# tum-vision/mem

Hardware: AMD Instinct MI355X
Metric: pretrain samples/sec (ViT-B, 224^2 event voxels) (higher is better)
Workload: dtype bf16

## Files before the change

include/memhip.h:

```cpp
#ifndef MEMHIP_H
#define MEMHIP_H

#include <stddef.h>
#include <stdint.h>

#ifdef __cplusplus
extern "C" {
#endif

#define MEMHIP_ABI_VERSION 7

#define MEMHIP_OK 0
#define MEMHIP_EINVAL (-1)
#define MEMHIP_EWORKSPACE (-2)
#define MEMHIP_ELAUNCH (-3)
#define MEMHIP_EUNSUPPORTED (-4)

typedef void* memhip_stream_t;

int memhip_abi_version(void);
const char* memhip_last_error(void);
const char* memhip_arch(void);
const char* memhip_build_flags(void);
int memhip_set_option(const char* name, int value);
// ... 126 lines not shown

#define MEMHIP_NT_128 0
#define MEMHIP_NT_G256 1
#define MEMHIP_NT_P8_256 2
#define MEMHIP_NT_P8_128 3
#define MEMHIP_NT_P8_PAIR 4
typedef struct memhip_nt_launch {
  int32_t kind;
  int32_t row0, rows;
  int32_t tail_rows;
  int32_t guard;
  int32_t copy;
  int32_t grid, tail_grid;
} memhip_nt_launch_t;
typedef struct memhip_nt_plan { int32_t count; memhip_nt_launch_t l[2]; } memhip_nt_plan_t;
int memhip_gemm_bf16_nt_plan(const memhip_gemm_args_t* args, int stream_cus, int device_cus, memhip_nt_plan_t* out);

int memhip_gemm_bf16_tn(const void* A, int64_t lda, const void* B, int64_t ldb, int R, int N, int K,
                        float* out, int64_t ldo, int accumulate, memhip_stream_t stream);
size_t memhip_gemm_bf16_tn_workspace(int R, int N, int K);
int memhip_gemm_bf16_tn_ws(const void* A, int64_t lda, const void* B, int64_t ldb, int R, int N, int K,
                           float* out, int64_t ldo, int accumulate, void* workspace, size_t workspace_bytes,
                           memhip_stream_t stream);
typedef struct memhip_tn_problem {
  const void* A; int64_t lda;
  const void* B; int64_t ldb;
  float* out; int64_t ldo;
  int32_t R, N, K;
  int32_t reserved0;
} memhip_tn_problem_t;
size_t memhip_gemm_bf16_tn_group_workspace(const memhip_tn_problem_t* problems, int count);
int memhip_gemm_bf16_tn_group(const memhip_tn_problem_t* problems, int count, int accumulate, void* workspace,
                              size_t workspace_bytes, memhip_stream_t stream);
int memhip_colsum_bf16(const void* in, int64_t ld, int R, int C, float* out, memhip_stream_t stream);
int memhip_colsum_fold(float* ws, int copies, int N, float* out, memhip_stream_t stream);

int memhip_residual_rows(const float* x, int64_t ldx, const int32_t* rows, const void* y, int64_t ldy, const float* gamma,
                         const float* rowkeep, float keep_prob, int R, int D, float* out, int64_t ldo,
                         memhip_stream_t stream);
int memhip_scatter_rows_f32(const float* src, int64_t lds, const int32_t* rows, int R, int D, float* dst, int64_t ldd,
                            memhip_stream_t stream);

int memhip_layernorm_fwd(const float* x, int64_t ldx, const int32_t* row_idx, int R, int D,
                         const float* gamma, const float* beta, float eps, void* y_bf16, int64_t ldy,
                         float* mean, float* rstd, memhip_stream_t stream);
int memhip_layernorm_bwd(const void* dy_bf16, int64_t lddy, const float* x, int64_t ldx,
                         const int32_t* row_idx, int R, int D, const float* gamma, const float* mean,
                         const float* rstd, float* dres, int64_t lddres, int accumulate, float* dgamma,
                         float* dbeta, memhip_stream_t stream);

int memhip_layerscale_grad(const void* W_bf16, int64_t ldw, const float* dW, int64_t lddw, const float* bias,
                           const float* dbias, const float* gamma, int N, int K, float* dgamma,
                           memhip_stream_t stream);

int memhip_layernorm_bwd_branch(const void* dy_bf16, int64_t lddy, const float* x, int64_t ldx, int R, int D,
                                const float* gamma, const float* mean, const float* rstd, float* dres,
                                int64_t lddres, float* dgamma, float* dbeta, const void* y_branch_bf16, int64_t ldyb,
                                const float* gamma_branch, const float* rowmask, float keep_prob,
                                int rows_per_sample, void* dy_branch_bf16, int64_t lddyb, float* dgamma_branch,
                                float* dbias_branch, memhip_stream_t stream);

int memhip_branch_bwd(const float* dx, int64_t lddx, const void* y_bf16, int64_t ldy, const float* gamma,
                      const float* rowmask, float keep_prob, int rows_per_sample, int M, int D,
                      void* dy_bf16, int64_t lddy, float* dgamma, float* dbias, memhip_stream_t stream);
int memhip_branch_bwd_map(const float* dx, int64_t lddx, const void* y_bf16, int64_t ldy, const float* gamma,
                          const float* rowmask, float keep_prob, int rows_per_sample, int M, int D,
// ... 170 lines not shown
```

mem_amd/csrc/common.h:

```cpp
#pragma once
#include <hip/hip_runtime.h>
#include <cstdarg>
#include <cstdio>
#include <cstdint>
#include "../../include/memhip.h"

namespace memhip {

extern thread_local char g_err[512];

inline int fail(int code, const char* fmt, ...) {
  va_list ap;
  va_start(ap, fmt);
  vsnprintf(g_err, sizeof(g_err), fmt, ap);
  va_end(ap);
  return code;
}

inline int check_launch(const char* what) {
  hipError_t e = hipGetLastError();
  if (e != hipSuccess) return fail(MEMHIP_ELAUNCH, "%s: %s", what, hipGetErrorString(e));
  return MEMHIP_OK;
}

enum { OPT_GEMM_P8, OPT_GEMM256, OPT_GEMM_SPLIT, OPT_GEMM_P8_HALF, OPT_GEMM_P8_MIN_N, OPT_GEMM256_MIN_N, OPT_TN_P8,
       OPT_RASTER_LDS, OPT_ATTN16, OPT_ATTN16_STAGGER, OPT_ATTN16_STAGGER_FWD, OPT_GEMM_STAGGER, OPT_GEMM_PREFETCH, OPT_RESERVE_CUS, OPT_LN_BWD_GRID, OPT_ATTN_WIN, OPT_GEMM_P8_PAIR, OPT_TN_GROUP, OPT_CONV_WAVES, OPT_RASTER_BANDS, OPT_COUNT_ };
int opt(int id);
int usable_cus(hipStream_t s = nullptr);
int max_cus();

inline hipStream_t as_stream(memhip_stream_t s) { return reinterpret_cast<hipStream_t>(s); }

inline int cdiv(long long a, long long b) { return (int)((a + b - 1) / b); }

}

#define MEMHIP_REQUIRE(cond, ...) \
  do { if (!(cond)) return memhip::fail(MEMHIP_EINVAL, __VA_ARGS__); } while (0)
#define MEMHIP_HIP(call) \
  do { hipError_t e_ = (call); if (e_ != hipSuccess) \
    return memhip::fail(MEMHIP_ELAUNCH, "%s: %s", #call, hipGetErrorString(e_)); } while (0)
```

mem_amd/csrc/core.cpp:

```cpp
#include "common.h"
#include <atomic>
#include <mutex>
#include <cstring>

namespace memhip {
thread_local char g_err[512] = "";

static std::atomic<int> g_opt[OPT_COUNT_] = {
     {1},  {1},  {1},  {1},  {512},
     {1024},  {1},  {1},  {1},  {40000},  {0},  {0},  {0},
     {0},  {2048},
     {1},
     {1},
     {1},
     {16},
     {0}};
static const char* const g_opt_name[OPT_COUNT_] = {"gemm_p8", "gemm256", "gemm_split", "gemm_p8_half", "gemm_p8_min_n",
                                                   "gemm256_min_n", "tn_p8", "raster_lds", "attn16", "attn16_stagger", "attn16_stagger_fwd", "gemm_stagger", "gemm_prefetch", "reserve_cus", "ln_bwd_grid", "attn_win", "gemm_p8_pair", "tn_group", "conv_waves", "raster_bands"};
int opt(int id) { return g_opt[id].load(std::memory_order_relaxed); }

struct StreamReserve { std::atomic<bool> used{false}; std::atomic<void*> stream{nullptr}; std::atomic<int> cus{0}; };
static StreamReserve g_reserve[32];
static int stream_reserved(hipStream_t s) {
  for (auto& r : g_reserve)
    if (r.used.load(std::memory_order_acquire) && r.stream.load(std::memory_order_relaxed) == (void*)s)
      return r.cus.load(std::memory_order_relaxed);
  return 0;
}

static int device_cu_count() {
  static std::atomic<int> device_cus{0};
  int n = device_cus.load(std::memory_order_relaxed);
  if (!n) {
    int dev = 0;
    hipDeviceProp_t prop;
    if (hipGetDevice(&dev) != hipSuccess || hipGetDeviceProperties(&prop, dev) != hipSuccess) return 0;
    n = prop.multiProcessorCount > 0 ? prop.multiProcessorCount : 256;
    device_cus.store(n, std::memory_order_relaxed);
  }
  return n;
}

int max_cus() { return device_cu_count(); }

int usable_cus(hipStream_t s) {
  const int n = device_cu_count();
  if (!n) return 0;
  int r = opt(OPT_RESERVE_CUS);
  const int rs = stream_reserved(s);
  r = r > rs ? r : rs;
  r = r < 0 ? 0 : (r + 7) / 8 * 8;
// ... 58 lines not shown
```

mem_amd/csrc/gemm_tn_p8.hip:

```cpp
#include <atomic>
#include "common.h"

#define P8_PRIO_MODE 0
#define P8_PRIO(x) __builtin_amdgcn_s_setprio(x)

namespace {

using namespace memhip;

constexpr int BM = 256, BN = 256, BR = 64;
constexpr int kThreads = 512;
constexpr int kHalf = BR * 128 * 2;
constexpr int kBuf = 4 * kHalf;
constexpr int kRing = 2 * kBuf;
enum { HA0 = 0, HA1 = 1, HB0 = 2, HB1 = 3 };

typedef __attribute__((ext_vector_type(8))) __bf16 bf16x8;
typedef __attribute__((ext_vector_type(4))) short s16x4;
typedef __attribute__((ext_vector_type(4))) float f32x4;
typedef __attribute__((ext_vector_type(16))) float f32x16;

__device__ __attribute__((aligned(256))) unsigned char g_tnp8_zero[256];
#ifdef P8_STAMP
__device__ unsigned long long g_tnp8_stamps[256 * 4];
#endif

__device__ __forceinline__ void glds16(const void* gsrc, void* lds_dst) {
  __builtin_amdgcn_global_load_lds((const __attribute__((address_space(1))) void*)gsrc,
                                   (__attribute__((address_space(3))) void*)lds_dst, 16, 0, 0);
}
#define P8_SADDR 1
__device__ __forceinline__ void glds16s(const void* sbase, unsigned voff, const void* lds_dst) {
  const unsigned lds = (unsigned)(unsigned long long)((const __attribute__((address_space(3))) char*)lds_dst);
  asm volatile("s_mov_b32 m0, %2\n\ts_nop 0\n\tglobal_load_lds_dwordx4 %0, %1" ::"v"(voff), "s"(sbase), "s"(lds) : "memory", "m0");
}
template <int OFF>
__device__ __forceinline__ s16x4 lds_tr16_b64(unsigned lds_addr) {
  s16x4 r;
  asm volatile("ds_read_b64_tr_b16 %0, %1 offset:%2" : "=v"(r) : "v"(lds_addr), "n"(OFF) : "memory");
  return r;
}
template <int OFF>
__device__ __forceinline__ bf16x8 tr_pair(unsigned lds_addr) {
  union { struct { s16x4 l, h; } s; bf16x8 v; } u;
  u.s.l = lds_tr16_b64<OFF>(lds_addr);
  u.s.h = lds_tr16_b64<OFF + 16 * 256>(lds_addr);
  return u.v;
}

#define TP_WAIT_VM() asm volatile("s_waitcnt vmcnt(10)" ::: "memory")
#define TP_BARRIER()                      \
  do {                                    \
    __builtin_amdgcn_sched_barrier(0);    \
    __builtin_amdgcn_s_barrier();         \
    __builtin_amdgcn_sched_barrier(0);    \
  } while (0)

__device__ __forceinline__ int tn_xcd_wid() {
  const int gq = (int)gridDim.x / 8, gr = (int)gridDim.x % 8, xcd = (int)blockIdx.x % 8;
  return (xcd < gr ? xcd * (gq + 1) : gr * (gq + 1) + (xcd - gr) * gq) + (int)blockIdx.x / 8;
}

template <bool WS>
__device__ __forceinline__ void tn_p8_body(const __bf16* __restrict__ A, long long lda, const __bf16* __restrict__ B,
                                           long long ldb, int R, int N, int K, float* __restrict__ out, long long ldo,
                                           int rows_per_split, int wid) {
  extern __shared__ __attribute__((aligned(16))) char smem[];
  const int lane = threadIdx.x & 63;
  const int wave = __builtin_amdgcn_readfirstlane(threadIdx.x >> 6);
  const int wr = wave >> 2, wc = wave & 3;
  const int ntk = K / BN;
  const int tiles = (N / BM) * ntk;
  const int tile = wid % tiles, sp = wid / tiles;
  const int n0 = (tile / ntk) * BM, k0 = (tile % ntk) * BN;
  const int rbeg = sp * rows_per_split;
  int rend = rbeg + rows_per_split;
  rend = rend < R ? rend : R;
  if (rbeg >= rend) return;
  const int total = ((rend - rbeg + 2 * BR - 1) / (2 * BR)) * 2;

  int prow[2];
  unsigned offA[2], offB[2];
  const int cpos = lane & 15;
#pragma unroll
  for (int j = 0; j < 2; ++j) {
    prow[j] = (wave * 2 + j) * 4 + (lane >> 4);
    const unsigned chunk = (unsigned)((((cpos >> 1) ^ (prow[j] & 7)) << 1) | (cpos & 1));
    offA[j] = (unsigned)((long long)prow[j] * lda * 2) + chunk * 16;
    offB[j] = (unsigned)((long long)prow[j] * ldb * 2) + chunk * 16;
  }
  const char* zsrc = reinterpret_cast<const char*>(g_tnp8_zero) + cpos * 16;
  auto stage = [&](int H, int buf, int g) {
    char* slot = smem + buf * kBuf + H * kHalf + wave * 2048;
    const int r0 = rbeg + g * BR;
    const bool isA = H == HA0 || H == HA1;
    const int c0 = (isA ? n0 : k0) + ((H == HA1 || H == HB1) ? 128 : 0);
    const char* base = reinterpret_cast<const char*>(isA ? A : B) + ((long long)r0 * (isA ? lda : ldb) + c0) * 2;
    if (r0 + BR <= rend) {
#pragma unroll
      for (int j = 0; j < 2; ++j) {
        if (P8_SADDR) glds16s(base, isA ? offA[j] : offB[j], slot + j * 1024);
        else glds16(base + (isA ? offA[j] : offB[j]), slot + j * 1024);
      }
    } else {
#pragma unroll
      for (int j = 0; j < 2; ++j) {
        const char* src = (r0 + prow[j] < rend) ? base + (isA ? offA[j] : offB[j]) : zsrc;
        glds16(src, slot + j * 1024);
      }
    }
  };
// ... 80 lines not shown
    TP_MFMA(2, bq0);                                                                                      \
    TP_BARRIER();                                                                                         \
  } while (0)

  TP_READ_B(bx, 0, 0);
#ifdef P8_STAMP
  if (wave == 0) {
    unsigned long long t_, r_;
    asm volatile("s_memtime %0\n\ts_memrealtime %1\n\ts_waitcnt lgkmcnt(0)" : "=s"(t_), "=s"(r_)::"memory");
    if (lane == 0) { g_tnp8_stamps[(blockIdx.x & 255) * 4 + 0] = t_; g_tnp8_stamps[(blockIdx.x & 255) * 4 + 1] = r_; }
  }
#endif
  for (int c = 0; c < total; c += 2) {
    {
      constexpr int bc = 0;
      TP_KTILE(bx, by);
    }
    {
      constexpr int bc = 1;
      TP_KTILE(by, bx);
    }
  }
#ifdef P8_STAMP
  if (wave == 0) {
    unsigned long long t_, r_;
    asm volatile("s_memtime %0\n\ts_memrealtime %1\n\ts_waitcnt lgkmcnt(0)" : "=s"(t_), "=s"(r_)::"memory");
    if (lane == 0) { g_tnp8_stamps[(blockIdx.x & 255) * 4 + 2] = t_; g_tnp8_stamps[(blockIdx.x & 255) * 4 + 3] = r_; }
  }
#endif
  if (wr == 0) TP_BARRIER();
  asm volatile("s_waitcnt vmcnt(0)" ::: "memory");
  TP_BARRIER();

  float* wreg = reinterpret_cast<float*>(smem + wave * 4096);
  const int kcol = k0 + (lane >> 5) * 128 + wc * 32 + (lane & 31);
  float* dst = WS ? out + (long long)sp * N * ldo : out;
#pragma unroll
  for (int i = 0; i < 2; ++i)
#pragma unroll
    for (int nf = 0; nf < 4; ++nf) {
#pragma unroll
      for (int j = 0; j < 2; ++j)
#pragma unroll
        for (int kf = 0; kf < 2; ++kf)
#pragma unroll
          for (int r = 0; r < 4; ++r) {
            const int row = (lane >> 4) * 4 + r;
            wreg[row * 64 + ((j * 32 + kf * 16 + (lane & 15)) ^ (((row >> 2) & 1) << 4))] = TP_ACC_EL(i * 2 + j, nf, kf, r);
          }
      const int nrow = n0 + i * 128 + wr * 64 + nf * 16;
      if constexpr (WS) {
#pragma unroll
        for (int it = 0; it < 4; ++it) {
          const int row = it * 4 + (lane >> 4), c4 = (lane & 15) * 4;
          *reinterpret_cast<float4*>(dst + (long long)(nrow + row) * ldo + k0 + (c4 >> 5) * 128 + wc * 32 + (c4 & 31)) =
              *reinterpret_cast<const float4*>(wreg + row * 64 + (c4 ^ (((row >> 2) & 1) << 4)));
        }
      } else {
#pragma unroll
        for (int row = 0; row < 16; ++row) {
          const float v = wreg[row * 64 + (lane ^ (((row >> 2) & 1) << 4))];
          atomicAdd(dst + (long long)(nrow + row) * ldo + kcol, v);
        }
      }
    }
}

template <bool WS>
__global__ __launch_bounds__(kThreads) void gemm_tn_p8_kernel(const __bf16* __restrict__ A, long long lda,
                                                              const __bf16* __restrict__ B, long long ldb,
                                                              int R, int N, int K, float* __restrict__ out,
                                                              long long ldo, int rows_per_split) {
  tn_p8_body<WS>(A, lda, B, ldb, R, N, K, out, ldo, rows_per_split, tn_xcd_wid());
}

constexpr int kTnGroupMax = 4;
struct TnGroupProblem {
  const __bf16* A;
  const __bf16* B;
  float* ws;
  float* out;
  long long lda, ldb, ldo;
  int R, N, K;
  int rows_per_split, splits;
  int wg_begin;
  int quad_begin;
};
struct TnGroup {
  TnGroupProblem p[kTnGroupMax];
  int count;
};
__global__ __launch_bounds__(kThreads) void gemm_tn_p8_group_kernel(const TnGroup g) {
  const int wid = tn_xcd_wid();
  int i = 0;
#pragma unroll
  for (int j = 1; j < kTnGroupMax; ++j)
    if (j < g.count && wid >= g.p[j].wg_begin) i = j;
  const TnGroupProblem& q = g.p[i];
  tn_p8_body<true>(q.A, q.lda, q.B, q.ldb, q.R, q.N, q.K, q.ws, (long long)q.K, q.rows_per_split, wid - q.wg_begin);
}
__global__ __launch_bounds__(256) void tn_reduce_group_kernel(const TnGroup g, int accumulate) {
  const int quad = blockIdx.x * 256 + threadIdx.x;
  int i = 0;
#pragma unroll
  for (int j = 1; j < kTnGroupMax; ++j)
    if (j < g.count && quad >= g.p[j].quad_begin) i = j;
  const TnGroupProblem& q = g.p[i];
  const long long i4 = (long long)(quad - q.quad_begin) * 4;
  const long long slab = (long long)q.N * q.K;
  if (i4 >= slab) return;
  float4 a = *reinterpret_cast<const float4*>(q.ws + i4);
  for (int s = 1; s < q.splits; ++s) {
    const float4 b = *reinterpret_cast<const float4*>(q.ws + s * slab + i4);
    a.x += b.x; a.y += b.y; a.z += b.z; a.w += b.w;
  }
  const long long n = i4 / q.K, k = i4 - n * q.K;
  float4* o = reinterpret_cast<float4*>(q.out + n * q.ldo + k);
  if (accumulate) {
    const float4 c = *o;
    a.x += c.x; a.y += c.y; a.z += c.z; a.w += c.w;
  }
  *o = a;
}

__global__ __launch_bounds__(256) void tn_reduce_kernel(const float* __restrict__ ws, int S, long long slab, int N, int K,
                                                        float* __restrict__ out, long long ldo, int accumulate) {
  const long long i4 = ((long long)blockIdx.x * 256 + threadIdx.x) * 4;
  if (i4 >= (long long)N * K) return;
  float4 a = *reinterpret_cast<const float4*>(ws + i4);
  for (int s = 1; s < S; ++s) {
    const float4 b = *reinterpret_cast<const float4*>(ws + s * slab + i4);
    a.x += b.x; a.y += b.y; a.z += b.z; a.w += b.w;
  }
  const long long n = i4 / K, k = i4 - n * K;
  float4* o = reinterpret_cast<float4*>(out + n * ldo + k);
  if (accumulate) {
    const float4 c = *o;
    a.x += c.x; a.y += c.y; a.z += c.z; a.w += c.w;
  }
  *o = a;
}

}

#ifdef P8_STAMP
extern "C" int memhip_debug_tnp8_stamps(unsigned long long* host_out) {
  return hipMemcpyFromSymbol(host_out, HIP_SYMBOL(g_tnp8_stamps), sizeof(unsigned long long) * 256 * 4) == hipSuccess ? 0 : -1;
}
#endif

namespace memhip {

static void tn_p8_plan(int R, int N, int K, int num_cu, int& tiles, int& splits, int& rows_per_split) {
  tiles = (N / BM) * (K / BN);
  const int pairs = cdiv(R, 2 * BR);
  splits = num_cu / tiles;
  if (splits < 1) splits = 1;
  if (splits > pairs / 2) splits = pairs / 2 > 0 ? pairs / 2 : 1;
  rows_per_split = cdiv(pairs, splits) * 2 * BR;
  splits = cdiv(R, rows_per_split);
}
static int tn_p8_num_cu(hipStream_t s = nullptr) { return usable_cus(s); }

size_t gemm_tn_p8_workspace(int R, int N, int K) {
  if (N % BM != 0 || K % BN != 0 || R < 2048) return 0;
  const int num_cu = max_cus();
  if (!num_cu) return 0;
  size_t need = 0;
  for (int cu = num_cu; cu >= 8; cu -= 8) {
    int tiles, splits, rps;
    tn_p8_plan(R, N, K, cu, tiles, splits, rps);
    const size_t b = splits > 1 ? (size_t)splits * N * K * sizeof(float) : 0;
    need = b > need ? b : need;
  }
  return need;
}

int gemm_tn_p8_dispatch(const void* A, long long lda, const void* B, long long ldb, int R, int N, int K, float* out,
                        long long ldo, int accumulate, float* ws, size_t ws_bytes, hipStream_t s) {
  if (N % BM != 0 || K % BN != 0 || R < 2048) return MEMHIP_EUNSUPPORTED;
  const int num_cu = tn_p8_num_cu(s);
  if (!num_cu) return MEMHIP_EUNSUPPORTED;
  int tiles, splits, rows_per_split;
  tn_p8_plan(R, N, K, num_cu, tiles, splits, rows_per_split);
  static std::atomic<bool> attr_done{false};
  if (!attr_done) {
    hipError_t e = hipFuncSetAttribute(reinterpret_cast<const void*>(gemm_tn_p8_kernel<false>),
                                       hipFuncAttributeMaxDynamicSharedMemorySize, kRing);
    if (e == hipSuccess)
      e = hipFuncSetAttribute(reinterpret_cast<const void*>(gemm_tn_p8_kernel<true>),
                              hipFuncAttributeMaxDynamicSharedMemorySize, kRing);
    if (e != hipSuccess) return fail(MEMHIP_ELAUNCH, "gemm_tn_p8: set smem attr: %s", hipGetErrorString(e));
    attr_done = true;
  }
  const size_t need = (size_t)splits * N * K * sizeof(float);
  if (ws && splits > 1 && ws_bytes >= need && ((uintptr_t)ws & 15) == 0 && ldo % 4 == 0 && ((uintptr_t)out & 15) == 0) {
    hipLaunchKernelGGL(gemm_tn_p8_kernel<true>, dim3(tiles * splits), dim3(kThreads), kRing, s, (const __bf16*)A, lda,
                       (const __bf16*)B, ldb, R, N, K, ws, (long long)K, rows_per_split);
    const long long quads = (long long)N * K / 4;
    hipLaunchKernelGGL(tn_reduce_kernel, dim3((unsigned)((quads + 255) / 256)), dim3(256), 0, s, ws, splits,
                       (long long)N * K, N, K, out, ldo, accumulate);
    return check_launch("gemm_bf16_tn(p8, workspace)");
  }
  if (!accumulate) {
    hipError_t e = hipMemset2DAsync(out, (size_t)ldo * sizeof(float), 0, (size_t)K * sizeof(float), (size_t)N, s);
    if (e != hipSuccess) return fail(MEMHIP_ELAUNCH, "gemm_tn_p8: memset: %s", hipGetErrorString(e));
  }
  hipLaunchKernelGGL(gemm_tn_p8_kernel<false>, dim3(tiles * splits), dim3(kThreads), kRing, s, (const __bf16*)A, lda,
                     (const __bf16*)B, ldb, R, N, K, out, ldo, rows_per_split);
  return check_launch("gemm_bf16_tn(p8)");
}

static bool tn_group_plan(const memhip_tn_problem_t* pr, int count, int num_cu, TnGroup& g, int& total_wgs, int& total_quads,
                          size_t& ws_floats) {
  if (count < 2 || count > kTnGroupMax || !num_cu) return false;
  int tiles_total = 0;
  for (int i = 0; i < count; ++i) {
    if (pr[i].N % BM != 0 || pr[i].K % BN != 0 || pr[i].R < 2048 || pr[i].ldo % 4 != 0 || ((uintptr_t)pr[i].out & 15) != 0) return false;
    tiles_total += (pr[i].N / BM) * (pr[i].K / BN);
  }
  int best_s = 0;
  double best_eff = 0.0;
  for (int r = 1; r <= 4; ++r) {
    const int sp = (r * num_cu) / tiles_total;
    if (sp < 2) continue;
    const double eff = (double)tiles_total * sp / ((double)r * num_cu);
    if (eff > best_eff + 1e-9) { best_eff = eff; best_s = sp; }
    if (eff >= 0.80) break;
  }
  if (best_s < 2) return false;
  total_wgs = 0; total_quads = 0; ws_floats = 0;
  g.count = count;
  for (int i = 0; i < count; ++i) {
    TnGroupProblem& q = g.p[i];
    const int tiles = (pr[i].N / BM) * (pr[i].K / BN);
    const int pairs = cdiv(pr[i].R, 2 * BR);
    int sp = best_s;
    if (sp > pairs / 2) sp = pairs / 2 > 0 ? pairs / 2 : 1;
    q.rows_per_split = cdiv(pairs, sp) * 2 * BR;
    q.splits = cdiv(pr[i].R, q.rows_per_split);
    q.A = (const __bf16*)pr[i].A; q.B = (const __bf16*)pr[i].B;
    q.lda = pr[i].lda; q.ldb = pr[i].ldb; q.ldo = pr[i].ldo;
    q.R = pr[i].R; q.N = pr[i].N; q.K = pr[i].K;
    q.out = pr[i].out;
    q.ws = nullptr;
    q.wg_begin = total_wgs;
    q.quad_begin = total_quads;
    total_wgs += tiles * q.splits;
    total_quads += (int)(((long long)pr[i].N * pr[i].K / 4 + 255) / 256 * 256);
    ws_floats += (size_t)q.splits * pr[i].N * pr[i].K;
  }
  return true;
}

size_t gemm_tn_p8_group_workspace(const memhip_tn_problem_t* pr, int count) {
  const int num_cu = max_cus();
  size_t need = 0;
  for (int cu = num_cu; cu >= 8; cu -= 8) {
    TnGroup g;
    int wgs, quads;
    size_t fl;
    if (tn_group_plan(pr, count, cu, g, wgs, quads, fl) && fl * sizeof(float) > need) need = fl * sizeof(float);
  }
  return need;
}

int gemm_tn_p8_group_dispatch(const memhip_tn_problem_t* pr, int count, int accumulate, float* ws, size_t ws_bytes, hipStream_t s) {
  TnGroup g;
  int wgs, quads;
  size_t fl;
  if (!ws || ((uintptr_t)ws & 15) != 0 || !tn_group_plan(pr, count, tn_p8_num_cu(s), g, wgs, quads, fl) ||
      fl * sizeof(float) > ws_bytes)
    return MEMHIP_EUNSUPPORTED;
  static std::atomic<bool> attr_done{false};
  if (!attr_done) {
    const hipError_t e = hipFuncSetAttribute(reinterpret_cast<const void*>(gemm_tn_p8_group_kernel),
                                             hipFuncAttributeMaxDynamicSharedMemorySize, kRing);
    if (e != hipSuccess) return fail(MEMHIP_ELAUNCH, "gemm_tn_p8(group): set smem attr: %s", hipGetErrorString(e));
    attr_done = true;
  }
  float* w = ws;
  for (int i = 0; i < count; ++i) {
    g.p[i].ws = w;
    w += (size_t)g.p[i].splits * g.p[i].N * g.p[i].K;
  }
  hipLaunchKernelGGL(gemm_tn_p8_group_kernel, dim3(wgs), dim3(kThreads), kRing, s, g);
  hipLaunchKernelGGL(tn_reduce_group_kernel, dim3((unsigned)(quads / 256)), dim3(256), 0, s, g, accumulate);
  return check_launch("gemm_bf16_tn_group(p8)");
}

}
```

Measured before the change: 7484.

## Schedule TN weight-gradient GEMM work from a host-built segment table

Replaces the fixed split-K grouping of TN (weight-gradient) GEMMs with a host-side planner. The planner emits a per-workgroup table of (product, tile, row range, slot) segments, which is cached per shape set and uploaded to the device once. Each workgroup can now process several segments and writes partial results into per-slot tile buffers. A table-driven reduction then sums each tile's slots. An optional 'even' mode (off by default) balances row-pair work across CUs exactly, while the default slice mode reproduces the old split scheme through the table. The cost is an extra table lookup and an indirection in the reduce.

```diff
diff --git a/include/memhip.h b/include/memhip.h
--- a/include/memhip.h
+++ b/include/memhip.h
@@ -182,6 +182,10 @@
 size_t memhip_gemm_bf16_tn_group_workspace(const memhip_tn_problem_t* problems, int count);
 int memhip_gemm_bf16_tn_group(const memhip_tn_problem_t* problems, int count, int accumulate, void* workspace,
                               size_t workspace_bytes, memhip_stream_t stream);
+typedef struct memhip_tn_segment { int32_t wg, product, tile, pair_begin, pair_end, slot; } memhip_tn_segment_t;
+typedef struct memhip_tn_tile_slots { int32_t product, tile, first_slot, count; } memhip_tn_tile_slots_t;
+int memhip_gemm_bf16_tn_plan(const int32_t* shapes, int count, int cus, int even, memhip_tn_segment_t* segments, int segment_cap,
+                             memhip_tn_tile_slots_t* tiles, int tile_cap, int32_t* info);
 int memhip_colsum_bf16(const void* in, int64_t ld, int R, int C, float* out, memhip_stream_t stream);
 int memhip_colsum_fold(float* ws, int copies, int N, float* out, memhip_stream_t stream);
 
diff --git a/mem_amd/csrc/common.h b/mem_amd/csrc/common.h
--- a/mem_amd/csrc/common.h
+++ b/mem_amd/csrc/common.h
@@ -24,7 +24,7 @@
 }
 
 enum { OPT_GEMM_P8, OPT_GEMM256, OPT_GEMM_SPLIT, OPT_GEMM_P8_HALF, OPT_GEMM_P8_MIN_N, OPT_GEMM256_MIN_N, OPT_TN_P8,
-       OPT_RASTER_LDS, OPT_ATTN16, OPT_ATTN16_STAGGER, OPT_ATTN16_STAGGER_FWD, OPT_GEMM_STAGGER, OPT_GEMM_PREFETCH, OPT_RESERVE_CUS, OPT_LN_BWD_GRID, OPT_ATTN_WIN, OPT_GEMM_P8_PAIR, OPT_TN_GROUP, OPT_CONV_WAVES, OPT_RASTER_BANDS, OPT_COUNT_ };
+       OPT_RASTER_LDS, OPT_ATTN16, OPT_ATTN16_STAGGER, OPT_ATTN16_STAGGER_FWD, OPT_GEMM_STAGGER, OPT_GEMM_PREFETCH, OPT_RESERVE_CUS, OPT_LN_BWD_GRID, OPT_ATTN_WIN, OPT_GEMM_P8_PAIR, OPT_TN_GROUP, OPT_CONV_WAVES, OPT_RASTER_BANDS, OPT_TN_EVEN, OPT_COUNT_ };
 int opt(int id);
 int usable_cus(hipStream_t s = nullptr);
 int max_cus();
diff --git a/mem_amd/csrc/core.cpp b/mem_amd/csrc/core.cpp
--- a/mem_amd/csrc/core.cpp
+++ b/mem_amd/csrc/core.cpp
@@ -14,9 +14,10 @@
      {1},
      {1},
      {16},
+     {0},
      {0}};
 static const char* const g_opt_name[OPT_COUNT_] = {"gemm_p8", "gemm256", "gemm_split", "gemm_p8_half", "gemm_p8_min_n",
-                                                   "gemm256_min_n", "tn_p8", "raster_lds", "attn16", "attn16_stagger", "attn16_stagger_fwd", "gemm_stagger", "gemm_prefetch", "reserve_cus", "ln_bwd_grid", "attn_win", "gemm_p8_pair", "tn_group", "conv_waves", "raster_bands"};
+                                                   "gemm256_min_n", "tn_p8", "raster_lds", "attn16", "attn16_stagger", "attn16_stagger_fwd", "gemm_stagger", "gemm_prefetch", "reserve_cus", "ln_bwd_grid", "attn_win", "gemm_p8_pair", "tn_group", "conv_waves", "raster_bands", "tn_even"};
 int opt(int id) { return g_opt[id].load(std::memory_order_relaxed); }
 
 struct StreamReserve { std::atomic<bool> used{false}; std::atomic<void*> stream{nullptr}; std::atomic<int> cus{0}; };
diff --git a/mem_amd/csrc/gemm_tn_p8.hip b/mem_amd/csrc/gemm_tn_p8.hip
--- a/mem_amd/csrc/gemm_tn_p8.hip
+++ b/mem_amd/csrc/gemm_tn_p8.hip
@@ -1,5 +1,9 @@
 #include <atomic>
+#include <memory>
+#include <mutex>
+#include <vector>
 #include "common.h"
+#include "gemm_tn_plan.hpp"
 
 #define P8_PRIO_MODE 0
 #define P8_PRIO(x) __builtin_amdgcn_s_setprio(x)
@@ -63,20 +67,12 @@
 
 template <bool WS>
 __device__ __forceinline__ void tn_p8_body(const __bf16* __restrict__ A, long long lda, const __bf16* __restrict__ B,
-                                           long long ldb, int R, int N, int K, float* __restrict__ out, long long ldo,
-                                           int rows_per_split, int wid) {
+                                           long long ldb, int n0, int k0, int rbeg, int rend, float* __restrict__ dst,
+                                           long long ldo) {
   extern __shared__ __attribute__((aligned(16))) char smem[];
   const int lane = threadIdx.x & 63;
   const int wave = __builtin_amdgcn_readfirstlane(threadIdx.x >> 6);
   const int wr = wave >> 2, wc = wave & 3;
-  const int ntk = K / BN;
-  const int tiles = (N / BM) * ntk;
-  const int tile = wid % tiles, sp = wid / tiles;
-  const int n0 = (tile / ntk) * BM, k0 = (tile % ntk) * BN;
-  const int rbeg = sp * rows_per_split;
-  int rend = rbeg + rows_per_split;
-  rend = rend < R ? rend : R;
-  if (rbeg >= rend) return;
   const int total = ((rend - rbeg + 2 * BR - 1) / (2 * BR)) * 2;
 
   int prow[2];
@@ -223,9 +219,10 @@
   asm volatile("s_waitcnt vmcnt(0)" ::: "memory");
   TP_BARRIER();
 
+  int le = lane;
+  asm volatile("" : "+v"(le));
   float* wreg = reinterpret_cast<float*>(smem + wave * 4096);
-  const int kcol = k0 + (lane >> 5) * 128 + wc * 32 + (lane & 31);
-  float* dst = WS ? out + (long long)sp * N * ldo : out;
+  const int kcol = (le >> 5) * 128 + wc * 32 + (le & 31);
 #pragma unroll
   for (int i = 0; i < 2; ++i)
 #pragma unroll
@@ -236,59 +233,77 @@
         for (int kf = 0; kf < 2; ++kf)
 #pragma unroll
           for (int r = 0; r < 4; ++r) {
-            const int row = (lane >> 4) * 4 + r;
-            wreg[row * 64 + ((j * 32 + kf * 16 + (lane & 15)) ^ (((row >> 2) & 1) << 4))] = TP_ACC_EL(i * 2 + j, nf, kf, r);
+            const int row = (le >> 4) * 4 + r;
+            wreg[row * 64 + ((j * 32 + kf * 16 + (le & 15)) ^ (((row >> 2) & 1) << 4))] = TP_ACC_EL(i * 2 + j, nf, kf, r);
           }
-      const int nrow = n0 + i * 128 + wr * 64 + nf * 16;
+      const int nrow = i * 128 + wr * 64 + nf * 16;
       if constexpr (WS) {
 #pragma unroll
         for (int it = 0; it < 4; ++it) {
-          const int row = it * 4 + (lane >> 4), c4 = (lane & 15) * 4;
-          *reinterpret_cast<float4*>(dst + (long long)(nrow + row) * ldo + k0 + (c4 >> 5) * 128 + wc * 32 + (c4 & 31)) =
+          const int row = it * 4 + (le >> 4), c4 = (le & 15) * 4;
+          *reinterpret_cast<float4*>(dst + (long long)(nrow + row) * ldo + (c4 >> 5) * 128 + wc * 32 + (c4 & 31)) =
               *reinterpret_cast<const float4*>(wreg + row * 64 + (c4 ^ (((row >> 2) & 1) << 4)));
         }
       } else {
 #pragma unroll
         for (int row = 0; row < 16; ++row) {
-          const float v = wreg[row * 64 + (lane ^ (((row >> 2) & 1) << 4))];
+          const float v = wreg[row * 64 + (le ^ (((row >> 2) & 1) << 4))];
           atomicAdd(dst + (long long)(nrow + row) * ldo + kcol, v);
         }
       }
     }
 }
 
-template <bool WS>
 __global__ __launch_bounds__(kThreads) void gemm_tn_p8_kernel(const __bf16* __restrict__ A, long long lda,
                                                               const __bf16* __restrict__ B, long long ldb,
                                                               int R, int N, int K, float* __restrict__ out,
                                                               long long ldo, int rows_per_split) {
-  tn_p8_body<WS>(A, lda, B, ldb, R, N, K, out, ldo, rows_per_split, tn_xcd_wid());
+  const int wid = tn_xcd_wid();
+  const int ntk = K / BN;
+  const int tiles = (N / BM) * ntk;
+  const int tile = wid % tiles, sp = wid / tiles;
+  const int n0 = (tile / ntk) * BM, k0 = (tile % ntk) * BN;
+  const int rbeg = sp * rows_per_split;
+  int rend = rbeg + rows_per_split;
+  rend = rend < R ? rend : R;
+  if (rbeg >= rend) return;
+  tn_p8_body<false>(A, lda, B, ldb, n0, k0, rbeg, rend, out + (long long)n0 * ldo + k0, ldo);
 }
 
 constexpr int kTnGroupMax = 4;
+constexpr int kSlotFloats = BM * BN;
 struct TnGroupProblem {
   const __bf16* A;
   const __bf16* B;
-  float* ws;
   float* out;
   long long lda, ldb, ldo;
   int R, N, K;
-  int rows_per_split, splits;
-  int wg_begin;
+  int tile_begin;
   int quad_begin;
 };
 struct TnGroup {
   TnGroupProblem p[kTnGroupMax];
   int count;
+  int max_seg, tile_off;
+  const int* table;
+  float* ws;
 };
 __global__ __launch_bounds__(kThreads) void gemm_tn_p8_group_kernel(const TnGroup g) {
   const int wid = tn_xcd_wid();
-  int i = 0;
-#pragma unroll
-  for (int j = 1; j < kTnGroupMax; ++j)
-    if (j < g.count && wid >= g.p[j].wg_begin) i = j;
-  const TnGroupProblem& q = g.p[i];
-  tn_p8_body<true>(q.A, q.lda, q.B, q.ldb, q.R, q.N, q.K, q.ws, (long long)q.K, q.rows_per_split, wid - q.wg_begin);
+  const int* seg = g.table + (long long)wid * g.max_seg * 8;
+  const int send = __builtin_amdgcn_readfirstlane(seg[6]);
+  for (int s = 0; s < send; ++s, seg += 8) {
+    const int i = __builtin_amdgcn_readfirstlane(seg[0]);
+    const int n0 = __builtin_amdgcn_readfirstlane(seg[1]), k0 = __builtin_amdgcn_readfirstlane(seg[2]);
+    const int rbeg = __builtin_amdgcn_readfirstlane(seg[3]), rend = __builtin_amdgcn_readfirstlane(seg[4]);
+    const int slot = __builtin_amdgcn_readfirstlane(seg[5]);
+    const TnGroupProblem& q = g.p[i];
+    tn_p8_body<true>(q.A, q.lda, q.B, q.ldb, n0, k0, rbeg, rend, g.ws + (long long)slot * kSlotFloats, (long long)BN);
+    if (s + 1 < send) {
+      asm volatile("s_waitcnt vmcnt(0)" ::: "memory");
+      TP_BARRIER();
+    }
+  }
 }
 __global__ __launch_bounds__(256) void tn_reduce_group_kernel(const TnGroup g, int accumulate) {
   const int quad = blockIdx.x * 256 + threadIdx.x;
@@ -298,15 +313,16 @@
     if (j < g.count && quad >= g.p[j].quad_begin) i = j;
   const TnGroupProblem& q = g.p[i];
   const long long i4 = (long long)(quad - q.quad_begin) * 4;
-  const long long slab = (long long)q.N * q.K;
-  if (i4 >= slab) return;
-  float4 a = *reinterpret_cast<const float4*>(q.ws + i4);
-  for (int s = 1; s < q.splits; ++s) {
-    const float4 b = *reinterpret_cast<const float4*>(q.ws + s * slab + i4);
+  if (i4 >= (long long)q.N * q.K) return;
+  const int n = (int)(i4 / q.K), k = (int)(i4 - (long long)n * q.K);
+  const int2 sl = *reinterpret_cast<const int2*>(g.table + g.tile_off + 2 * (q.tile_begin + (n / BM) * (q.K / BN) + k / BN));
+  const float* src = g.ws + (long long)sl.x * kSlotFloats + (n % BM) * BN + (k % BN);
+  float4 a = *reinterpret_cast<const float4*>(src);
+  for (int s = 1; s < sl.y; ++s) {
+    const float4 b = *reinterpret_cast<const float4*>(src + (long long)s * kSlotFloats);
     a.x += b.x; a.y += b.y; a.z += b.z; a.w += b.w;
   }
-  const long long n = i4 / q.K, k = i4 - n * q.K;
-  float4* o = reinterpret_cast<float4*>(q.out + n * q.ldo + k);
+  float4* o = reinterpret_cast<float4*>(q.out + (long long)n * q.ldo + k);
   if (accumulate) {
     const float4 c = *o;
     a.x += c.x; a.y += c.y; a.z += c.z; a.w += c.w;
@@ -314,24 +330,6 @@
   *o = a;
 }
 
-__global__ __launch_bounds__(256) void tn_reduce_kernel(const float* __restrict__ ws, int S, long long slab, int N, int K,
-                                                        float* __restrict__ out, long long ldo, int accumulate) {
-  const long long i4 = ((long long)blockIdx.x * 256 + threadIdx.x) * 4;
-  if (i4 >= (long long)N * K) return;
-  float4 a = *reinterpret_cast<const float4*>(ws + i4);
-  for (int s = 1; s < S; ++s) {
-    const float4 b = *reinterpret_cast<const float4*>(ws + s * slab + i4);
-    a.x += b.x; a.y += b.y; a.z += b.z; a.w += b.w;
-  }
-  const long long n = i4 / K, k = i4 - n * K;
-  float4* o = reinterpret_cast<float4*>(out + n * ldo + k);
-  if (accumulate) {
-    const float4 c = *o;
-    a.x += c.x; a.y += c.y; a.z += c.z; a.w += c.w;
-  }
-  *o = a;
-}
-
 }
 
 #ifdef P8_STAMP
@@ -341,6 +339,139 @@
 #endif
 
 namespace memhip {
+
+static int tn_p8_num_cu(hipStream_t s = nullptr) { return usable_cus(s); }
+
+namespace {
+struct TnTable {
+  int device, count, cus, even;
+  TnShape sh[kTnGroupMax];
+  int wgs, slots, max_seg, tile_off;
+  int tile_begin[kTnGroupMax];
+  bool split;
+  std::vector<int> host;
+  int* dev = nullptr;
+  hipEvent_t ready = nullptr;
+  hipStream_t upload_stream = nullptr;
+  bool landed = false;
+};
+std::mutex g_tab_mu;
+std::vector<std::unique_ptr<TnTable>> g_tabs;
+
+const TnTable* tn_table(const TnShape* sh, int count, int cus, int even, hipStream_t s, int* rc) {
+  int device = 0;
+  if (hipGetDevice(&device) != hipSuccess) { *rc = fail(MEMHIP_ELAUNCH, "gemm_tn_p8: hipGetDevice"); return nullptr; }
+  std::lock_guard<std::mutex> lock(g_tab_mu);
+  TnTable* t = nullptr;
+  for (auto& e : g_tabs) {
+    if (e->device != device || e->count != count || e->cus != cus || e->even != even) continue;
+    bool same = true;
+    for (int i = 0; i < count; ++i) same = same && e->sh[i].R == sh[i].R && e->sh[i].N == sh[i].N && e->sh[i].K == sh[i].K;
+    if (same) { t = e.get(); break; }
+  }
+  if (!t) {
+    const TnPlan plan = gemm_tn_plan(sh, count, cus, even != 0);
+    if (!plan.workgroups) { *rc = MEMHIP_EUNSUPPORTED; return nullptr; }
+    std::unique_ptr<TnTable> e(new TnTable);
+    e->device = device; e->count = count; e->cus = cus; e->even = even;
+    for (int i = 0; i < count; ++i) e->sh[i] = sh[i];
+    e->wgs = plan.workgroups;
+    e->slots = plan.slots;
+    e->split = plan.slots > (int)plan.tiles.size();
+    e->max_seg = plan.max_segments;
+    e->tile_off = 8 * plan.workgroups * plan.max_segments;
+    e->host.assign(e->tile_off + 2 * plan.tiles.size(), 0);
+    for (int w = 0; w < plan.workgroups; ++w)
+      for (int k = plan.wg_begin[w]; k < plan.wg_begin[w + 1]; ++k) {
+        const TnSegment& g = plan.segments[k];
+        const int ntk = sh[g.product].K / BN, rend = g.pair_end * 2 * BR;
+        int* o = &e->host[8 * (w * plan.max_segments + k - plan.wg_begin[w])];
+        o[0] = g.product; o[1] = (g.tile / ntk) * BM; o[2] = (g.tile % ntk) * BN;
+        o[3] = g.pair_begin * 2 * BR; o[4] = rend < sh[g.product].R ? rend : sh[g.product].R; o[5] = g.slot;
+        o[6] = plan.wg_begin[w + 1] - plan.wg_begin[w];
+      }
+    for (size_t k = 0; k < plan.tiles.size(); ++k) {
+      if (plan.tiles[k].tile == 0) e->tile_begin[plan.tiles[k].product] = (int)k;
+      e->host[e->tile_off + 2 * k] = plan.tiles[k].first_slot;
+      e->host[e->tile_off + 2 * k + 1] = plan.tiles[k].count;
+    }
+    hipError_t err = hipMalloc(reinterpret_cast<void**>(&e->dev), e->host.size() * sizeof(int));
+    if (err == hipSuccess) err = hipEventCreateWithFlags(&e->ready, hipEventDisableTiming);
+    if (err == hipSuccess) err = hipMemcpyAsync(e->dev, e->host.data(), e->host.size() * sizeof(int), hipMemcpyHostToDevice, s);
+    if (err == hipSuccess) err = hipEventRecord(e->ready, s);
+    if (err != hipSuccess) {
+      if (e->ready) (void)hipEventDestroy(e->ready);
+      if (e->dev) (void)hipFree(e->dev);
+      *rc = fail(MEMHIP_ELAUNCH, "gemm_tn_p8: plan upload: %s", hipGetErrorString(err));
+      return nullptr;
+    }
+    e->upload_stream = s;
+    t = e.get();
+    g_tabs.push_back(std::move(e));
+  } else if (!t->landed) {
+    if (hipEventQuery(t->ready) == hipSuccess) t->landed = true;
+    else if (s != t->upload_stream && hipStreamWaitEvent(s, t->ready, 0) != hipSuccess) {
+      *rc = fail(MEMHIP_ELAUNCH, "gemm_tn_p8: wait for the plan upload");
+      return nullptr;
+    }
+  }
+  return t;
+}
+
+bool tn_shapes(const memhip_tn_problem_t* pr, int count, TnShape* sh) {
+  if (count < 1 || count > kTnGroupMax) return false;
+  for (int i = 0; i < count; ++i) {
+    sh[i] = TnShape{pr[i].R, pr[i].N, pr[i].K};
+    if (!tn_shape_fits(sh[i])) return false;
+  }
+  return true;
+}
+
+int tn_balanced_launch(const memhip_tn_problem_t* pr, int count, int accumulate, float* ws, size_t ws_bytes, bool need_split,
+                       hipStream_t s) {
+  TnShape sh[kTnGroupMax];
+  const int cus = tn_p8_num_cu(s);
+  if (!ws || ((uintptr_t)ws & 15) != 0 || !cus || !tn_shapes(pr, count, sh)) return MEMHIP_EUNSUPPORTED;
+  for (int i = 0; i < count; ++i)
+    if (pr[i].ldo % 4 != 0 || ((uintptr_t)pr[i].out & 15) != 0) return MEMHIP_EUNSUPPORTED;
+  int rc = MEMHIP_EUNSUPPORTED;
+  const TnTable* t = tn_table(sh, count, cus, opt(OPT_TN_EVEN) != 0, s, &rc);
+  if (!t) return rc;
+  if ((size_t)t->slots * kSlotFloats * sizeof(float) > ws_bytes || (need_split && !t->split)) return MEMHIP_EUNSUPPORTED;
+  static std::atomic<bool> attr_done{false};
+  if (!attr_done) {
+    const hipError_t e = hipFuncSetAttribute(reinterpret_cast<const void*>(gemm_tn_p8_group_kernel),
+                                             hipFuncAttributeMaxDynamicSharedMemorySize, kRing);
+    if (e != hipSuccess) return fail(MEMHIP_ELAUNCH, "gemm_tn_p8(workspace): set smem attr: %s", hipGetErrorString(e));
+    attr_done = true;
+  }
+  TnGroup g = {};
+  g.count = count;
+  g.max_seg = t->max_seg; g.tile_off = t->tile_off;
+  g.table = t->dev;
+  g.ws = ws;
+  long long quads = 0;
+  for (int i = 0; i < count; ++i) {
+    TnGroupProblem& q = g.p[i];
+    q.A = (const __bf16*)pr[i].A; q.B = (const __bf16*)pr[i].B; q.out = pr[i].out;
+    q.lda = pr[i].lda; q.ldb = pr[i].ldb; q.ldo = pr[i].ldo;
+    q.R = pr[i].R; q.N = pr[i].N; q.K = pr[i].K;
+    q.tile_begin = t->tile_begin[i];
+    q.quad_begin = (int)quads;
+    quads += ((long long)pr[i].N * pr[i].K / 4 + 255) / 256 * 256;
+  }
+  if (quads > 0x7fffffff) return MEMHIP_EUNSUPPORTED;
+  hipLaunchKernelGGL(gemm_tn_p8_group_kernel, dim3(t->wgs), dim3(kThreads), kRing, s, g);
+  hipLaunchKernelGGL(tn_reduce_group_kernel, dim3((unsigned)(quads / 256)), dim3(256), 0, s, g, accumulate);
+  return check_launch("gemm_bf16_tn(p8, workspace)");
+}
+
+size_t tn_slots_bytes(const TnShape* sh, int count, bool* split) {
+  const int num_cu = max_cus();
+  if (!num_cu) return 0;
+  return (size_t)gemm_tn_plan_max_slots(sh, count, num_cu, split) * kSlotFloats * sizeof(float);
+}
+}
 
 static void tn_p8_plan(int R, int N, int K, int num_cu, int& tiles, int& splits, int& rows_per_split) {
   tiles = (N / BM) * (K / BN);
@@ -351,20 +482,12 @@
   rows_per_split = cdiv(pairs, splits) * 2 * BR;
   splits = cdiv(R, rows_per_split);
 }
-static int tn_p8_num_cu(hipStream_t s = nullptr) { return usable_cus(s); }
 
 size_t gemm_tn_p8_workspace(int R, int N, int K) {
-  if (N % BM != 0 || K % BN != 0 || R < 2048) return 0;
-  const int num_cu = max_cus();
-  if (!num_cu) return 0;
-  size_t need = 0;
-  for (int cu = num_cu; cu >= 8; cu -= 8) {
-    int tiles, splits, rps;
-    tn_p8_plan(R, N, K, cu, tiles, splits, rps);
-    const size_t b = splits > 1 ? (size_t)splits * N * K * sizeof(float) : 0;
-    need = b > need ? b : need;
-  }
-  return need;
+  const TnShape sh{R, N, K};
+  bool split = false;
+  const size_t bytes = tn_slots_bytes(&sh, 1, &split);
+  return split ? bytes : 0;
 }
 
 int gemm_tn_p8_dispatch(const void* A, long long lda, const void* B, long long ldb, int R, int N, int K, float* out,
@@ -372,112 +495,60 @@
   if (N % BM != 0 || K % BN != 0 || R < 2048) return MEMHIP_EUNSUPPORTED;
   const int num_cu = tn_p8_num_cu(s);
   if (!num_cu) return MEMHIP_EUNSUPPORTED;
+  if (ws) {
+    memhip_tn_problem_t q = {};
+    q.A = A; q.lda = lda; q.B = B; q.ldb = ldb; q.out = out; q.ldo = ldo; q.R = R; q.N = N; q.K = K;
+    const int rc = tn_balanced_launch(&q, 1, accumulate, ws, ws_bytes, true, s);
+    if (rc != MEMHIP_EUNSUPPORTED) return rc;
+  }
   int tiles, splits, rows_per_split;
   tn_p8_plan(R, N, K, num_cu, tiles, splits, rows_per_split);
   static std::atomic<bool> attr_done{false};
   if (!attr_done) {
-    hipError_t e = hipFuncSetAttribute(reinterpret_cast<const void*>(gemm_tn_p8_kernel<false>),
-                                       hipFuncAttributeMaxDynamicSharedMemorySize, kRing);
-    if (e == hipSuccess)
-      e = hipFuncSetAttribute(reinterpret_cast<const void*>(gemm_tn_p8_kernel<true>),
-                              hipFuncAttributeMaxDynamicSharedMemorySize, kRing);
+    const hipError_t e = hipFuncSetAttribute(reinterpret_cast<const void*>(gemm_tn_p8_kernel),
+                                             hipFuncAttributeMaxDynamicSharedMemorySize, kRing);
     if (e != hipSuccess) return fail(MEMHIP_ELAUNCH, "gemm_tn_p8: set smem attr: %s", hipGetErrorString(e));
     attr_done = true;
-  }
-  const size_t need = (size_t)splits * N * K * sizeof(float);
-  if (ws && splits > 1 && ws_bytes >= need && ((uintptr_t)ws & 15) == 0 && ldo % 4 == 0 && ((uintptr_t)out & 15) == 0) {
-    hipLaunchKernelGGL(gemm_tn_p8_kernel<true>, dim3(tiles * splits), dim3(kThreads), kRing, s, (const __bf16*)A, lda,
-                       (const __bf16*)B, ldb, R, N, K, ws, (long long)K, rows_per_split);
-    const long long quads = (long long)N * K / 4;
-    hipLaunchKernelGGL(tn_reduce_kernel, dim3((unsigned)((quads + 255) / 256)), dim3(256), 0, s, ws, splits,
-                       (long long)N * K, N, K, out, ldo, accumulate);
-    return check_launch("gemm_bf16_tn(p8, workspace)");
   }
   if (!accumulate) {
     hipError_t e = hipMemset2DAsync(out, (size_t)ldo * sizeof(float), 0, (size_t)K * sizeof(float), (size_t)N, s);
     if (e != hipSuccess) return fail(MEMHIP_ELAUNCH, "gemm_tn_p8: memset: %s", hipGetErrorString(e));
   }
-  hipLaunchKernelGGL(gemm_tn_p8_kernel<false>, dim3(tiles * splits), dim3(kThreads), kRing, s, (const __bf16*)A, lda,
+  hipLaunchKernelGGL(gemm_tn_p8_kernel, dim3(tiles * splits), dim3(kThreads), kRing, s, (const __bf16*)A, lda,
                      (const __bf16*)B, ldb, R, N, K, out, ldo, rows_per_split);
   return check_launch("gemm_bf16_tn(p8)");
 }
 
-static bool tn_group_plan(const memhip_tn_problem_t* pr, int count, int num_cu, TnGroup& g, int& total_wgs, int& total_quads,
-                          size_t& ws_floats) {
-  if (count < 2 || count > kTnGroupMax || !num_cu) return false;
-  int tiles_total = 0;
-  for (int i = 0; i < count; ++i) {
-    if (pr[i].N % BM != 0 || pr[i].K % BN != 0 || pr[i].R < 2048 || pr[i].ldo % 4 != 0 || ((uintptr_t)pr[i].out & 15) != 0) return false;
-    tiles_total += (pr[i].N / BM) * (pr[i].K / BN);
-  }
-  int best_s = 0;
-  double best_eff = 0.0;
-  for (int r = 1; r <= 4; ++r) {
-    const int sp = (r * num_cu) / tiles_total;
-    if (sp < 2) continue;
-    const double eff = (double)tiles_total * sp / ((double)r * num_cu);
-    if (eff > best_eff + 1e-9) { best_eff = eff; best_s = sp; }
-    if (eff >= 0.80) break;
-  }
-  if (best_s < 2) return false;
-  total_wgs = 0; total_quads = 0; ws_floats = 0;
-  g.count = count;
-  for (int i = 0; i < count; ++i) {
-    TnGroupProblem& q = g.p[i];
-    const int tiles = (pr[i].N / BM) * (pr[i].K / BN);
-    const int pairs = cdiv(pr[i].R, 2 * BR);
-    int sp = best_s;
-    if (sp > pairs / 2) sp = pairs / 2 > 0 ? pairs / 2 : 1;
-    q.rows_per_split = cdiv(pairs, sp) * 2 * BR;
-    q.splits = cdiv(pr[i].R, q.rows_per_split);
-    q.A = (const __bf16*)pr[i].A; q.B = (const __bf16*)pr[i].B;
-    q.lda = pr[i].lda; q.ldb = pr[i].ldb; q.ldo = pr[i].ldo;
-    q.R = pr[i].R; q.N = pr[i].N; q.K = pr[i].K;
-    q.out = pr[i].out;
-    q.ws = nullptr;
-    q.wg_begin = total_wgs;
-    q.quad_begin = total_quads;
-    total_wgs += tiles * q.splits;
-    total_quads += (int)(((long long)pr[i].N * pr[i].K / 4 + 255) / 256 * 256);
-    ws_floats += (size_t)q.splits * pr[i].N * pr[i].K;
-  }
-  return true;
-}
-
 size_t gemm_tn_p8_group_workspace(const memhip_tn_problem_t* pr, int count) {
-  const int num_cu = max_cus();
-  size_t need = 0;
-  for (int cu = num_cu; cu >= 8; cu -= 8) {
-    TnGroup g;
-    int wgs, quads;
-    size_t fl;
-    if (tn_group_plan(pr, count, cu, g, wgs, quads, fl) && fl * sizeof(float) > need) need = fl * sizeof(float);
-  }
-  return need;
+  TnShape sh[kTnGroupMax];
+  if (count < 2 || !tn_shapes(pr, count, sh)) return 0;
+  return tn_slots_bytes(sh, count, nullptr);
 }
 
 int gemm_tn_p8_group_dispatch(const memhip_tn_problem_t* pr, int count, int accumulate, float* ws, size_t ws_bytes, hipStream_t s) {
-  TnGroup g;
-  int wgs, quads;
-  size_t fl;
-  if (!ws || ((uintptr_t)ws & 15) != 0 || !tn_group_plan(pr, count, tn_p8_num_cu(s), g, wgs, quads, fl) ||
-      fl * sizeof(float) > ws_bytes)
-    return MEMHIP_EUNSUPPORTED;
-  static std::atomic<bool> attr_done{false};
-  if (!attr_done) {
-    const hipError_t e = hipFuncSetAttribute(reinterpret_cast<const void*>(gemm_tn_p8_group_kernel),
-                                             hipFuncAttributeMaxDynamicSharedMemorySize, kRing);
-    if (e != hipSuccess) return fail(MEMHIP_ELAUNCH, "gemm_tn_p8(group): set smem attr: %s", hipGetErrorString(e));
-    attr_done = true;
-  }
-  float* w = ws;
-  for (int i = 0; i < count; ++i) {
-    g.p[i].ws = w;
-    w += (size_t)g.p[i].splits * g.p[i].N * g.p[i].K;
-  }
-  hipLaunchKernelGGL(gemm_tn_p8_group_kernel, dim3(wgs), dim3(kThreads), kRing, s, g);
-  hipLaunchKernelGGL(tn_reduce_group_kernel, dim3((unsigned)(quads / 256)), dim3(256), 0, s, g, accumulate);
-  return check_launch("gemm_bf16_tn_group(p8)");
-}
-
-}
+  if (count < 2) return MEMHIP_EUNSUPPORTED;
+  return tn_balanced_launch(pr, count, accumulate, ws, ws_bytes, false, s);
+}
+
+}
+
+extern "C" int memhip_gemm_bf16_tn_plan(const int32_t* shapes, int count, int cus, int even, memhip_tn_segment_t* segments,
+                                        int segment_cap, memhip_tn_tile_slots_t* tiles, int tile_cap, int32_t* info) {
+  MEMHIP_REQUIRE(shapes && info && count >= 1 && count <= kTnGroupMax && cus >= 1,
+                 "gemm_tn_plan: 1..4 products, cus >= 1");
+  memhip::TnShape sh[kTnGroupMax];
+  for (int i = 0; i < count; ++i) sh[i] = memhip::TnShape{shapes[3 * i], shapes[3 * i + 1], shapes[3 * i + 2]};
+  const memhip::TnPlan plan = memhip::gemm_tn_plan(sh, count, cus, even != 0);
+  info[0] = plan.workgroups; info[1] = plan.slots; info[2] = plan.max_segments; info[3] = plan.load_lo; info[4] = plan.load_hi;
+  info[5] = (int)plan.segments.size(); info[6] = (int)plan.tiles.size();
+  info[7] = memhip::gemm_tn_plan_max_slots(sh, count, cus, nullptr);
+  MEMHIP_REQUIRE((!segments || (int)plan.segments.size() <= segment_cap) && (!tiles || (int)plan.tiles.size() <= tile_cap),
+                 "gemm_tn_plan: %d segments / %d tiles do not fit the caller's arrays", info[5], info[6]);
+  for (size_t k = 0; segments && k < plan.segments.size(); ++k) {
+    const memhip::TnSegment& g = plan.segments[k];
+    segments[k] = memhip_tn_segment_t{g.wg, g.product, g.tile, g.pair_begin, g.pair_end, g.slot};
+  }
+  for (size_t k = 0; tiles && k < plan.tiles.size(); ++k)
+    tiles[k] = memhip_tn_tile_slots_t{plan.tiles[k].product, plan.tiles[k].tile, plan.tiles[k].first_slot, plan.tiles[k].count};
+  return MEMHIP_OK;
+}
diff --git a/mem_amd/csrc/gemm_tn_plan.cpp b/mem_amd/csrc/gemm_tn_plan.cpp
--- /dev/null
+++ b/mem_amd/csrc/gemm_tn_plan.cpp
@@ -0,0 +1,156 @@
+#include "gemm_tn_plan.hpp"
+
+#include <algorithm>
+
+namespace memhip {
+namespace {
+
+struct Piece { int product, tile, pb, pe, wg; };
+
+int piece_rows(const Piece& p, int R) {
+  const long long end = (long long)p.pe * kTnPairRows;
+  return (int)((end < R ? end : R) - (long long)p.pb * kTnPairRows);
+}
+
+}
+
+static TnPlan tn_slice_plan(const TnShape* sh, int count, int cus) {
+  TnPlan plan;
+  std::vector<int> T(count), P(count);
+  int tiles_total = 0;
+  for (int i = 0; i < count; ++i) {
+    T[i] = (sh[i].N / kTnTileDim) * (sh[i].K / kTnTileDim);
+    P[i] = (sh[i].R + kTnPairRows - 1) / kTnPairRows;
+    tiles_total += T[i];
+  }
+  int common = cus / tiles_total;
+  if (count > 1) {
+    double best_eff = 0.0;
+    common = 0;
+    for (int r = 1; r <= 4; ++r) {
+      const int sp = (int)((long long)r * cus / tiles_total);
+      if (sp < 2) continue;
+      const double eff = (double)tiles_total * sp / ((double)r * cus);
+      if (eff > best_eff + 1e-9) { best_eff = eff; common = sp; }
+      if (eff >= 0.80) break;
+    }
+    if (common < 2) return plan;
+  }
+  int wg = 0;
+  plan.load_lo = 1 << 30;
+  for (int i = 0; i < count; ++i) {
+    int sp = common < 1 ? 1 : common;
+    if (sp > P[i] / 2) sp = P[i] / 2 > 0 ? P[i] / 2 : 1;
+    const int per = (P[i] + sp - 1) / sp;
+    sp = (P[i] + per - 1) / per;
+    for (int t = 0; t < T[i]; ++t) plan.tiles.push_back({i, t, plan.slots + t * sp, sp});
+    for (int s = 0; s < sp; ++s)
+      for (int t = 0; t < T[i]; ++t, ++wg) {
+        const int pe = (s + 1) * per < P[i] ? (s + 1) * per : P[i];
+        plan.segments.push_back({wg, i, t, s * per, pe, plan.slots + t * sp + s});
+        plan.load_lo = std::min(plan.load_lo, pe - s * per);
+        plan.load_hi = std::max(plan.load_hi, pe - s * per);
+      }
+    plan.slots += T[i] * sp;
+  }
+  plan.workgroups = wg;
+  plan.max_segments = 1;
+  plan.wg_begin.resize(wg + 1);
+  for (int w = 0; w <= wg; ++w) plan.wg_begin[w] = w;
+  return plan;
+}
+
+TnPlan gemm_tn_plan(const TnShape* sh, int count, int cus, bool even) {
+  TnPlan plan;
+  if (count < 1 || cus < 1) return plan;
+  for (int i = 0; i < count; ++i)
+    if (!tn_shape_fits(sh[i])) return plan;
+  if (!even) return tn_slice_plan(sh, count, cus);
+  std::vector<int> T(count), P(count);
+  long long U = 0;
+  for (int i = 0; i < count; ++i) {
+    T[i] = (sh[i].N / kTnTileDim) * (sh[i].K / kTnTileDim);
+    P[i] = (sh[i].R + kTnPairRows - 1) / kTnPairRows;
+    U += (long long)T[i] * P[i];
+  }
+  const int G = (int)std::min<long long>(cus, U / 2);
+  const int qmax = (int)((U + G - 1) / G);
+  auto share = [&](int w) { return (int)((w + 1) * U / G - w * U / G); };
+  plan.load_lo = (int)(U / G);
+  plan.load_hi = qmax;
+
+  std::vector<std::vector<std::vector<Piece>>> pieces(count);
+  std::vector<std::vector<int>> pos(count);
+  int w = 0;
+  for (int i = 0; i < count; ++i) {
+    pieces[i].resize(T[i]);
+    pos[i].assign(T[i], 0);
+    int bands = P[i] / qmax;
+    const int rest = P[i] - bands * qmax;
+    if (bands > 0 && 2 * rest < qmax) --bands;
+    for (int b = 0; b < bands; ++b)
+      for (int t = 0; t < T[i]; ++t, ++w) {
+        const int len = share(w);
+        pieces[i][t].push_back({i, t, pos[i][t], pos[i][t] + len, w});
+        pos[i][t] += len;
+      }
+  }
+  int used = 0;
+  for (int i = 0; i < count; ++i)
+    for (int t = 0; t < T[i]; ++t)
+      while (pos[i][t] < P[i]) {
+        const int len = std::min(P[i] - pos[i][t], share(w) - used);
+        pieces[i][t].push_back({i, t, pos[i][t], pos[i][t] + len, w});
+        pos[i][t] += len;
+        used += len;
+        if (used == share(w)) { ++w; used = 0; }
+      }
+
+  for (int i = 0; i < count; ++i)
+    for (int t = 0; t < T[i]; ++t) {
+      std::vector<Piece> kept;
+      for (Piece p : pieces[i][t]) {
+        if (!kept.empty() && piece_rows(kept.back(), sh[i].R) < kTnMinRows) {
+          p.pb = kept.back().pb;
+          kept.pop_back();
+        }
+        kept.push_back(p);
+      }
+      if (kept.size() > 1 && piece_rows(kept.back(), sh[i].R) < kTnMinRows) {
+        const int pe = kept.back().pe;
+        kept.pop_back();
+        kept.back().pe = pe;
+      }
+      pieces[i][t].swap(kept);
+    }
+
+  for (int i = 0; i < count; ++i)
+    for (int t = 0; t < T[i]; ++t) {
+      plan.tiles.push_back({i, t, plan.slots, (int)pieces[i][t].size()});
+      for (const Piece& p : pieces[i][t]) plan.segments.push_back({p.wg, p.product, p.tile, p.pb, p.pe, plan.slots++});
+    }
+  std::stable_sort(plan.segments.begin(), plan.segments.end(),
+                   [](const TnSegment& a, const TnSegment& b) { return a.wg < b.wg; });
+  plan.workgroups = G;
+  plan.wg_begin.assign(G + 1, 0);
+  for (const TnSegment& s : plan.segments) ++plan.wg_begin[s.wg + 1];
+  for (int g = 0; g < G; ++g) {
+    plan.max_segments = std::max(plan.max_segments, plan.wg_begin[g + 1]);
+    plan.wg_begin[g + 1] += plan.wg_begin[g];
+  }
+  return plan;
+}
+
+int gemm_tn_plan_max_slots(const TnShape* shapes, int count, int device_cus, bool* split) {
+  int most = 0;
+  if (split) *split = false;
+  for (int cu = device_cus; cu >= 8; cu -= 8)
+    for (int even = 0; even < 2; ++even) {
+      const TnPlan p = gemm_tn_plan(shapes, count, cu, even != 0);
+      most = std::max(most, p.slots);
+      if (split && p.slots > (int)p.tiles.size()) *split = true;
+    }
+  return most;
+}
+
+}
diff --git a/mem_amd/csrc/gemm_tn_plan.hpp b/mem_amd/csrc/gemm_tn_plan.hpp
--- /dev/null
+++ b/mem_amd/csrc/gemm_tn_plan.hpp
@@ -0,0 +1,41 @@
+#pragma once
+#include <cstddef>
+#include <vector>
+
+namespace memhip {
+
+constexpr int kTnTileDim = 256;
+constexpr int kTnPairRows = 128;
+constexpr int kTnMinRows = 256;
+constexpr int kTnMinR = 2048;
+
+struct TnShape { int R, N, K; };
+
+struct TnSegment {
+  int wg;
+  int product, tile;
+  int pair_begin, pair_end;
+  int slot;
+};
+
+struct TnTileSlots { int product, tile, first_slot, count; };
+
+struct TnPlan {
+  int workgroups = 0;
+  int slots = 0;
+  int max_segments = 0;
+  int load_lo = 0, load_hi = 0;
+  std::vector<int> wg_begin;
+  std::vector<TnSegment> segments;
+  std::vector<TnTileSlots> tiles;
+};
+
+inline bool tn_shape_fits(const TnShape& s) {
+  return s.N > 0 && s.K > 0 && s.N % kTnTileDim == 0 && s.K % kTnTileDim == 0 && s.R >= kTnMinR;
+}
+
+TnPlan gemm_tn_plan(const TnShape* shapes, int count, int cus, bool even);
+
+int gemm_tn_plan_max_slots(const TnShape* shapes, int count, int device_cus, bool* split);
+
+}
```

Result: no change. 7446 (-0.5%).
